# theartful/polychase

Hardware: AMD Instinct MI355X
Metric: optical-flow frames/sec (higher is better)
Workload: dtype u8/int32 fixed-point + f32 2x2 solve; 1 GPU; C2 1920x1080 300-frame synthetic clip, 3-level pyramidal LK (max_level=3); width=1920, height=1080, max_level=3, window=10, pairs_per_frame=8, frames_per_gpu=1877, arith=opencv_x86, parallelism=single GPU

## Files before the change

polychase_amd/csrc/hip/kernels_gftt.hip:

```cpp
#include <algorithm>
#include <cstring>
#include <type_traits>
#include <rocprim/device/device_radix_sort.hpp>

#include <cmath>

#include "kernels.hpp"

namespace pc {

constexpr int TW = 64, TH = 16;
constexpr int CW = TW + 2, CH = TH + 2;

constexpr int ME_R = 8;
constexpr int ME_TW = 64, ME_TH = 2 * ME_R;

template <int SOBEL, bool MASKED>
__global__ __launch_bounds__(256) void min_eig_fused_kernel(const uint8_t* __restrict__ img, int pitch, int w, int h,
                                                            float* __restrict__ eig, GfttGrid g,
                                                            uint32_t* __restrict__ cell_max, float f1, float f0, int hi_prio,
                                                            const uint8_t* __restrict__ mask) {
    helper_priority(hi_prio);
    const int lane = threadIdx.x & 63, wave = threadIdx.x >> 6;
    const int tx0 = (blockIdx.x * 2 + (wave & 1)) * ME_TW, ty0 = (blockIdx.y * 2 + (wave >> 1)) * ME_TH;
    if (tx0 >= w || ty0 >= h) return;
    const int x = tx0 + 2 * (lane & 31), y0 = ty0 + ME_R * (lane >> 5);
    const bool lane_on = x < w && y0 < h;
    const int cx_lo = tx0 / g.cell_w, cx_hi = min(tx0 + ME_TW - 1, w - 1) / g.cell_w;
    const int cy_lo = ty0 / g.cell_h, cy_hi = min(ty0 + ME_TH - 1, h - 1) / g.cell_h;
    const bool one_cell = cx_lo == cx_hi && cy_lo == cy_hi;
    const bool four_regs = !one_cell && g.cell_w >= ME_TW && g.cell_h >= ME_TH;
    const int bx = (cx_lo + 1) * g.cell_w, by = (cy_lo + 1) * g.cell_h;
    uint32_t kmax[4] = {0u, 0u, 0u, 0u};
    const bool edge_tile = tx0 == 0 || ty0 == 0 || tx0 + ME_TW + 1 > w || ty0 + ME_TH + 1 > h;

    auto walk = [&](auto edge_tag) {
        constexpr bool edge = decltype(edge_tag)::value;
        const int a = (x - 2) & ~3;
        const uint32_t o8 = (uint32_t)(x - 2 - a) * 8u;
        const uint8_t* col = img + a;
        const int cw = w - (x - 1);
        float rx[3][4], ry[3][4];
        double hprev[3][2], acc[3][2];
        auto emit = [&](int y, const double (&sv)[3][2]) {
            float e[2];
#pragma unroll
            for (int j = 0; j < 2; j++) {
                const float a2 = (float)sv[0][j] * 0.5f;
                const float b2 = (float)sv[1][j];
                const float c2 = (float)sv[2][j] * 0.5f;
                const float t = a2 - c2;
                e[j] = (a2 + c2) - sqrtf(t * t + b2 * b2);
            }
            float* out = eig + (size_t)y * w + x;
            const bool two = x + 1 < w;
            if (two && ((w & 1) == 0)) {
                *reinterpret_cast<float2*>(out) = make_float2(e[0], e[1]);
            } else {
                out[0] = e[0];
                if (two) out[1] = e[1];
            }
            uint32_t k0 = float_to_ordered(e[0]), k1 = two ? float_to_ordered(e[1]) : 0u;
            if (MASKED) {
                const uint8_t* m = mask + (size_t)y * w + x;
                if ((w & 1) == 0) {
                    const uint32_t mm = *reinterpret_cast<const uint16_t*>(m);
                    if ((mm & 0xffu) == 0) k0 = 0u;
                    if ((mm >> 8) == 0) k1 = 0u;
                } else {
                    if (m[0] == 0) k0 = 0u;
                    if (two && m[1] == 0) k1 = 0u;
                }
            }
            if (one_cell) {
                kmax[0] = max(kmax[0], max(k0, k1));
            } else if (four_regs) {
                const int qy = y >= by ? 2 : 0;
#pragma unroll
                for (int q = 0; q < 4; q++) {
                    const uint32_t v0 = (qy + (x >= bx ? 1 : 0)) == q ? k0 : 0u;
                    const uint32_t v1 = (qy + (x + 1 >= bx ? 1 : 0)) == q ? k1 : 0u;
                    kmax[q] = max(kmax[q], max(v0, v1));
                }
            } else {
                atomicMax(&cell_max[(y / g.cell_h) * g.cols + x / g.cell_w], k0);
                if (two) atomicMax(&cell_max[(y / g.cell_h) * g.cols + (x + 1) / g.cell_w], k1);
            }
        };
#pragma unroll
        for (int k = 0; k < ME_R + 4; k++) {
            const int gy = min(y0 - 2 + k, h);
            const uint32_t d0 = *reinterpret_cast<const uint32_t*>(col + (ptrdiff_t)gy * pitch);
            const uint32_t d1 = *reinterpret_cast<const uint32_t*>(col + (ptrdiff_t)gy * pitch + 4);
            const uint32_t lo = __builtin_amdgcn_alignbit(d1, d0, o8), hi = d1 >> o8;
            float gv[6];
            gv[0] = (float)(lo & 0xffu);
            gv[1] = (float)((lo >> 8) & 0xffu);
// ... 229 lines not shown
                                                           const uint8_t* __restrict__ mask) {
    helper_priority(hi_prio);
    const int x = blockIdx.x * 64 + (threadIdx.x & 63), y = blockIdx.y * 4 + (threadIdx.x >> 6);
    if (x >= w || y >= h) return;
    const size_t n = (size_t)w * h;
    const int a0 = block / 2;
    double sxx = 0, sxy = 0, syy = 0;
    if (rows) {
        for (int j = 0; j < block; j++) {
            const size_t at = (size_t)reflect101(y + j - a0, h) * w + x;
            sxx += rows[at];
            sxy += rows[n + at];
            syy += rows[2 * n + at];
        }
    } else {
        for (int j = 0; j < block; j++) {
            const size_t row = (size_t)reflect101(y + j - a0, h) * w;
            double rxx = 0, rxy = 0, ryy = 0;
            for (int i = 0; i < block; i++) {
                const size_t at = row + reflect101(x + i - a0, w);
                rxx += (double)cov[at];
                rxy += (double)cov[n + at];
                ryy += (double)cov[2 * n + at];
            }
            sxx += rxx;
            sxy += rxy;
            syy += ryy;
        }
    }
    float e;
    if (harris) {
        const float a = (float)sxx, b = (float)sxy, c = (float)syy;
        const float ac = a * c, bb = b * b;
        const float det = ac - bb, tr = a + c;
        if (harris == 2 && x < (w / 4) * 4) {
            const float kt = (float)harris_k * tr;
            e = det - kt * tr;
        } else {
            e = (float)((double)det - harris_k * (double)tr * (double)tr);
        }
    } else {
        const float a = (float)sxx * 0.5f, b = (float)sxy, c = (float)syy * 0.5f;
        const float t = a - c;
        e = (a + c) - sqrtf(t * t + b * b);
    }
    eig[(size_t)y * w + x] = e;
    uint32_t key = float_to_ordered(e);
    if (MASKED && mask[(size_t)y * w + x] == 0) key = 0u;
    const int cell = (y / g.cell_h) * g.cols + x / g.cell_w;
    const int cell0 = __builtin_amdgcn_readfirstlane(cell);
    if (__all(cell == cell0)) {
#pragma unroll
        for (int d = 32; d >= 1; d >>= 1) key = max(key, (uint32_t)__shfl_xor((int)key, d));
        if ((threadIdx.x & 63) == (unsigned)(__ffsll((long long)__ballot(1)) - 1)) atomicMax(&cell_max[cell0], key);
    } else {
        atomicMax(&cell_max[cell], key);
    }
}

bool launch_corner_response(const Level& l0, float* eig, float* cov, double* box_rows, const GfttGrid& g, uint32_t* cell_max, int block_size, int gradient_size,
                            bool harris, double harris_k, int sobel_fma, hipStream_t s, const uint8_t* mask) {
    SobelTaps T;
    int taps = 0;
    if (!make_sobel_taps(gradient_size, block_size, &T, &taps)) return false;
    dim3 grid((l0.w + 63) / 64, (l0.h + 3) / 4);
    if (taps == 3)
        hipLaunchKernelGGL(cov_kernel<3>, grid, dim3(256), 0, s, l0.img, l0.pitch, l0.w, l0.h, cov, T, sobel_fma, helper_prio_arg());
    else if (taps == 5)
        hipLaunchKernelGGL(cov_kernel<5>, grid, dim3(256), 0, s, l0.img, l0.pitch, l0.w, l0.h, cov, T, sobel_fma, helper_prio_arg());
    else
        hipLaunchKernelGGL(cov_kernel<7>, grid, dim3(256), 0, s, l0.img, l0.pitch, l0.w, l0.h, cov, T, sobel_fma, helper_prio_arg());
    if (box_rows) hipLaunchKernelGGL(box_rows_kernel, grid, dim3(256), 0, s, cov, l0.w, l0.h, block_size, box_rows, helper_prio_arg());
    const int harris_mode = harris ? ((sobel_fma & 1) ? 2 : 1) : 0;
    if (mask)
        hipLaunchKernelGGL(box_response_kernel<true>, grid, dim3(256), 0, s, cov, (const double*)box_rows, l0.w, l0.h, block_size, harris_mode, harris_k, eig, g, cell_max,
                           helper_prio_arg(), mask);
    else
        hipLaunchKernelGGL(box_response_kernel<false>, grid, dim3(256), 0, s, cov, (const double*)box_rows, l0.w, l0.h, block_size, harris_mode, harris_k, eig, g, cell_max,
                           helper_prio_arg(), (const uint8_t*)nullptr);
    return true;
}

constexpr int NMS_SUB = 4;

struct SortRange {
    uint32_t hi, shift;
};
__host__ __device__ __forceinline__ SortRange make_sort_range(uint32_t lo, uint32_t hi) {
    SortRange r;
    r.hi = hi;
    r.shift = 0;
    const uint32_t span = hi > lo ? hi - lo : 0u;
    while ((span >> r.shift) >= (uint32_t)kSortBuckets) r.shift++;
    return r;
}
__device__ __forceinline__ uint32_t bucket_of(uint32_t ord, const SortRange& r) {
    const uint32_t d = r.hi > ord ? r.hi - ord : 0u;
    const uint32_t b = d >> r.shift;
    return b < (uint32_t)kSortBuckets ? b : (uint32_t)kSortBuckets - 1u;
}

template <bool MASKED>
__global__ __launch_bounds__(256) void nms_kernel(const float* __restrict__ eig, int w, int h, GfttGrid g,
                                                  const uint32_t* __restrict__ cell_max, double quality_level,
                                                  unsigned long long* __restrict__ keys, uint32_t cap,
                                                  uint32_t* __restrict__ counter, uint8_t* __restrict__ cstate,
                                                  uint32_t* __restrict__ sort_params, uint32_t* __restrict__ hist,
                                                  uint32_t* __restrict__ ticket, uint32_t* __restrict__ bucket_offsets,
                                                  uint32_t* __restrict__ bin_hist, int n_tiles,
                                                  unsigned long long* __restrict__ slots, uint32_t* __restrict__ zero, int zero_words,
                                                  int hi_prio, const uint8_t* __restrict__ mask) {
    helper_priority(hi_prio);
    __shared__ float s_thr[kMaxGridCells];
    __shared__ uint32_t s_hi, s_lo;
    __shared__ float s_v[CH][CW + 2];
    __shared__ uint32_t s_wave[4];
    __shared__ uint32_t s_base;
    const int tid = threadIdx.x;
    const int x0 = blockIdx.x * TW;
    const int ncells = g.rows * g.cols;
    if (tid == 0) {
        s_hi = 0u;
        s_lo = 0xffffffffu;
    }
    __syncthreads();
    for (int i = tid; i < ncells; i += 256) {
        const float mx = (MASKED && cell_max[i] == 0u) ? 0.f : ordered_to_float(cell_max[i]);
        s_thr[i] = (float)((double)mx * quality_level);
        atomicMax(&s_hi, cell_max[i]);
        atomicMin(&s_lo, float_to_ordered(s_thr[i] > 0.f ? s_thr[i] : 0.f));
    }
    __syncthreads();
    const SortRange range = make_sort_range(s_lo, s_hi);
    if (blockIdx.x == 0 && blockIdx.y == 0) {
        if (tid == 0) {
            sort_params[0] = range.hi;
            sort_params[1] = range.shift;
        }
        if (bin_hist)
            for (int i = tid; i < n_tiles; i += 256) bin_hist[i] = 0u;
    }
    for (int i = (blockIdx.y * gridDim.x + blockIdx.x) * 256 + tid; i < zero_words; i += gridDim.x * gridDim.y * 256) zero[i] = 0u;
    const int r = tid >> 4, q = tid & 15;
    const int x = x0 + 4 * q;
    uint32_t flags = 0;
    float vals[NMS_SUB][4];
#pragma unroll
    for (int sub = 0; sub < NMS_SUB; sub++) {
        const int y0 = (blockIdx.y * NMS_SUB + sub) * TH;
        const int y = y0 + r;
        __syncthreads();
        const bool big_cells = g.cell_w >= CW && g.cell_h >= CH;
        const int ccx0 = max(x0 - 1, 0) / g.cell_w, ccy0 = max(y0 - 1, 0) / g.cell_h;
        const int bx = (ccx0 + 1) * g.cell_w, by = (ccy0 + 1) * g.cell_h;
        auto thr_at = [&](int ax, int ay) -> float {
            const int cx = big_cells ? ccx0 + (ax >= bx) : ax / g.cell_w;
            const int cy = big_cells ? ccy0 + (ay >= by) : ay / g.cell_h;
            return s_thr[cy * g.cols + cx];
        };
        if (y0 < h) {
            float v[4] = {0.f, 0.f, 0.f, 0.f};
            if (y < h && x < w) {
                const float* row = eig + (size_t)y * w;
                if (x + 3 < w && (w & 3) == 0) {
                    const float4 e = *reinterpret_cast<const float4*>(row + x);
                    v[0] = e.x; v[1] = e.y; v[2] = e.z; v[3] = e.w;
                } else {
                    for (int i = 0; i < 4 && x + i < w; i++) v[i] = row[x + i];
                }
#pragma unroll
                for (int i = 0; i < 4; i++) v[i] = (x + i < w && v[i] > thr_at(x + i, y)) ? v[i] : 0.f;
            }
#pragma unroll
            for (int i = 0; i < 4; i++) s_v[r + 1][4 * q + 1 + i] = v[i];
            if (tid < 2 * CW + 2 * TH) {
                int cx, cy;
                if (tid < 2 * CW) {
                    cy = tid < CW ? 0 : CH - 1;
                    cx = tid < CW ? tid : tid - CW;
                } else {
                    const int k = tid - 2 * CW;
                    cy = 1 + (k >> 1);
                    cx = (k & 1) ? CW - 1 : 0;
                }
                const int ax = x0 - 1 + cx, ay = y0 - 1 + cy;
                float e = 0.f;
                if (ax >= 0 && ax < w && ay >= 0 && ay < h) {
                    e = eig[(size_t)ay * w + ax];
                    e = (e > thr_at(ax, ay)) ? e : 0.f;
                }
                s_v[cy][cx] = e;
            }
        }
        __syncthreads();
#pragma unroll
        for (int i = 0; i < 4; i++) vals[sub][i] = 0.f;
        if (y < h && x < w) {
            float cm[6];
#pragma unroll
            for (int i = 0; i < 6; i++) {
                const float a = s_v[r][4 * q + i], b = s_v[r + 1][4 * q + i], c = s_v[r + 2][4 * q + i];
                const float m = a > b ? a : b;
                cm[i] = m > c ? m : c;
            }
            uint32_t f4 = 0;
            uint32_t on = 0xfu;
            if (MASKED) {
                const uint8_t* mk = mask + (size_t)y * w + x;
                uint32_t m4 = 0;
                if (x + 3 < w && ((w & 3) == 0)) {
                    m4 = *reinterpret_cast<const uint32_t*>(mk);
                } else {
                    for (int i = 0; i < 4 && x + i < w; i++) m4 |= (uint32_t)mk[i] << (8 * i);
                }
                on = ((m4 & 0xffu) ? 1u : 0u) | ((m4 & 0xff00u) ? 2u : 0u) | ((m4 & 0xff0000u) ? 4u : 0u) | ((m4 & 0xff000000u) ? 8u : 0u);
            }
#pragma unroll
            for (int i = 0; i < 4; i++) {
                const float val = s_v[r + 1][4 * q + 1 + i];
                float m = cm[i] > cm[i + 1] ? cm[i] : cm[i + 1];
                m = m > cm[i + 2] ? m : cm[i + 2];
                const int xi = x + i;
                if (val != 0.f && val == m && xi >= 1 && xi < w - 1 && y >= 1 && y < h - 1 && (!MASKED || ((on >> i) & 1u))) {
                    f4 |= 1u << i;
                    vals[sub][i] = val;
                }
            }
            flags |= f4 << (4 * sub);
            uint8_t* cs = cstate + (size_t)y * w + x;
            if (x + 3 < w && ((w & 3) == 0)) {
                *reinterpret_cast<uint32_t*>(cs) = (f4 & 1u) | ((f4 & 2u) << 7) | ((f4 & 4u) << 14) | ((f4 & 8u) << 21);
            } else {
                for (int i = 0; i < 4 && x + i < w; i++) cs[i] = (uint8_t)((f4 >> i) & 1u);
            }
        }
    }
    const int lane = tid & 63, wave = tid >> 6;
    const uint32_t cnt = (uint32_t)__popc(flags);
    uint32_t incl = cnt;
#pragma unroll
    for (int d = 1; d < 64; d <<= 1) {
        const uint32_t t = __shfl_up(incl, d);
        if (lane >= d) incl += t;
    }
    if (lane == 63) s_wave[wave] = incl;
    __syncthreads();
    if (tid == 0) {
        const uint32_t total = s_wave[0] + s_wave[1] + s_wave[2] + s_wave[3];
        s_base = total ? atomicAdd(counter, total) : 0u;
    }
    __syncthreads();
    if (cnt != 0) {
        uint32_t pos = s_base + incl - cnt;
        for (int wv = 0; wv < wave; wv++) pos += s_wave[wv];
#pragma unroll
        for (int sub = 0; sub < NMS_SUB; sub++) {
            const int y = (blockIdx.y * NMS_SUB + sub) * TH + r;
#pragma unroll
            for (int i = 0; i < 4; i++) {
                if (flags & (1u << (4 * sub + i))) {
                    const uint32_t ord = float_to_ordered(vals[sub][i]);
                    if (pos < cap) {
                        const unsigned long long key = ((unsigned long long)ord << 32) | (unsigned long long)(uint32_t)(y * w + x + i);
                        const uint32_t b = bucket_of(ord, range);
                        if (slots) {
                            const uint32_t at = atomicAdd(&hist[b], 1u);
                            slots[(size_t)b * kBucketSlots + min(at, (uint32_t)kBucketSlots - 1u)] = key;
                        } else {
                            keys[pos] = key;
                            atomicAdd(&hist[b], 1u);
                        }
                    }
                    pos++;
                }
            }
        }
    }
    if (ticket && last_workgroup(ticket, gridDim.x * gridDim.y)) {
        __shared__ uint32_t s_scan[256];
        const uint32_t total = scan_exclusive_256_fixed<kSortBuckets / 256>(hist, bucket_offsets, s_scan);
        if (tid == 0) bucket_offsets[kSortBuckets] = total;
    }
}

void launch_nms(const float* eig, int w, int h, const GfttGrid& g, const uint32_t* cell_max, double quality_level,
                unsigned long long* keys, uint32_t cap, uint32_t* counter, uint8_t* cstate, uint32_t* sort_params, uint32_t* hist,
                uint32_t* ticket, uint32_t* bucket_offsets, uint32_t* bin_hist, hipStream_t s,
                unsigned long long* slots, uint32_t* zero, int zero_words, const uint8_t* mask) {
    dim3 grid((w + TW - 1) / TW, (h + NMS_SUB * TH - 1) / (NMS_SUB * TH));
    if (mask)
        hipLaunchKernelGGL(nms_kernel<true>, grid, dim3(256), 0, s, eig, w, h, g, cell_max, quality_level, keys, cap, counter, cstate,
                           sort_params, hist, ticket, bucket_offsets, bin_hist, bin_hist ? bin_num_tiles(w, h) : 0, slots, zero,
                           zero ? zero_words : 0, helper_prio_arg(), mask);
    else
        hipLaunchKernelGGL(nms_kernel<false>, grid, dim3(256), 0, s, eig, w, h, g, cell_max, quality_level, keys, cap, counter, cstate,
                           sort_params, hist, ticket, bucket_offsets, bin_hist, bin_hist ? bin_num_tiles(w, h) : 0, slots, zero,
                           zero ? zero_words : 0, helper_prio_arg(), (const uint8_t*)nullptr);
}

constexpr int kBucketLds = 512;

__global__ __launch_bounds__(256) void bucket_scatter_kernel(const unsigned long long* __restrict__ keys, uint32_t cap,
                                                             const uint32_t* __restrict__ counter, const uint32_t* __restrict__ sort_params,
                                                             const uint32_t* __restrict__ offsets, uint32_t* __restrict__ cursor,
                                                             unsigned long long* __restrict__ out, int hi_prio) {
    helper_priority(hi_prio);
    const uint32_t n = min(*counter, cap);
    SortRange range;
    range.hi = sort_params[0];
    range.shift = sort_params[1];
    for (uint32_t i = blockIdx.x * blockDim.x + threadIdx.x; i < n; i += gridDim.x * blockDim.x) {
        const unsigned long long key = keys[i];
        const uint32_t b = bucket_of((uint32_t)(key >> 32), range);
        out[offsets[b] + atomicAdd(&cursor[b], 1u)] = key;
    }
}

constexpr int kBucketsPerWave = 4;

constexpr int kSortWaves = 4;
static_assert(kBucketSlots == kBucketLds, "a bucket beyond its slots is a bucket beyond the fast path");
template <bool SLOTS>
__global__ __launch_bounds__(64 * kSortWaves) void bucket_sort_kernel(const unsigned long long* __restrict__ in, const uint32_t* __restrict__ offsets,
                                                         unsigned long long* __restrict__ out, uint32_t* __restrict__ overflow, int hi_prio) {
    helper_priority(hi_prio);
    __shared__ unsigned long long s_all[kSortWaves][kBucketLds];
    const int lane = threadIdx.x & 63, wave = threadIdx.x >> 6;
    unsigned long long* const s_keys = s_all[wave];
    const int b0 = (blockIdx.x * kSortWaves + wave) * kBucketsPerWave;
    if (b0 >= kSortBuckets) return;
    uint32_t o[kBucketsPerWave + 1];
#pragma unroll
    for (int k = 0; k <= kBucketsPerWave; k++) o[k] = offsets[min(b0 + k, kSortBuckets)];
    const uint32_t lo = o[0], n4 = o[kBucketsPerWave] - lo;
    if (n4 == 0) return;
    if (n4 <= (uint32_t)kBucketLds) {
        unsigned long long ld[kBucketLds / 64];
#pragma unroll
        for (int q = 0; q < kBucketLds / 64; q++) {
            const uint32_t i = lane + 64 * q;
            size_t at = lo + i;
            if (SLOTS) {
                int k = 0;
#pragma unroll
                for (int kk = 1; kk < kBucketsPerWave; kk++)
                    if (lo + i >= o[kk]) k = kk;
                at = (size_t)(b0 + k) * kBucketSlots + (lo + i - o[k]);
            }
            ld[q] = i < n4 ? in[at] : 0ull;
        }
#pragma unroll
        for (int q = 0; q < kBucketLds / 64; q++) {
            const uint32_t i = lane + 64 * q;
            if (i < n4) s_keys[i] = ld[q];
        }
        __builtin_amdgcn_fence(__ATOMIC_ACQ_REL, "wavefront");
        uint32_t longest = 0;
#pragma unroll
// ... 2 lines not shown
            const unsigned long long mine = s_keys[i];
            uint32_t a = lo, b = o[1];
#pragma unroll
            for (int k = 1; k < kBucketsPerWave; k++)
                if (lo + i >= o[k]) {
                    a = o[k];
                    b = o[k + 1];
                }
            const uint32_t first = a - lo, len = b - a;
            uint32_t rank = 0;
#pragma unroll 8
            for (uint32_t j = 0; j < longest; j++) {
                const unsigned long long other = s_keys[first + min(j, len - 1u)];
                rank += (j < len && other > mine) ? 1u : 0u;
            }
            out[a + rank] = mine;
        }
        return;
    }
    for (int b = b0; b < b0 + kBucketsPerWave && b < kSortBuckets; b++) {
        const uint32_t base = offsets[b], n = offsets[b + 1] - base;
        const unsigned long long* const src = SLOTS ? in + (size_t)b * kBucketSlots : in + base;
        if (n == 0) continue;
        if (n > (uint32_t)kBucketLds) {
            if (lane == 0) atomicOr(overflow, 1u);
            for (uint32_t i = lane; i < n; i += 64) out[base + i] = src[SLOTS ? min(i, (uint32_t)kBucketSlots - 1u) : i];
            continue;
        }
        __builtin_amdgcn_fence(__ATOMIC_ACQ_REL, "wavefront");
        for (uint32_t i = lane; i < n; i += 64) s_keys[i] = src[i];
        __builtin_amdgcn_fence(__ATOMIC_ACQ_REL, "wavefront");
        for (uint32_t i = lane; i < n; i += 64) {
            const unsigned long long mine = s_keys[i];
            uint32_t rank = 0;
#pragma unroll 8
            for (uint32_t j = 0; j < n; j++) rank += s_keys[j] > mine ? 1u : 0u;
            out[base + rank] = mine;
        }
    }
}

void launch_bucket_sort(const unsigned long long* keys, uint32_t cap, uint32_t n_launch, const uint32_t* counter, const uint32_t* sort_params,
                        const uint32_t* offsets, uint32_t* cursor, unsigned long long* scratch, unsigned long long* out,
                        uint32_t* overflow, hipStream_t s) {
    const unsigned blocks = std::max(1u, std::min<unsigned>(1024u, (n_launch + 255u) / 256u));
    hipLaunchKernelGGL(bucket_scatter_kernel, dim3(blocks), dim3(256), 0, s, keys, cap, counter, sort_params, offsets, cursor, scratch, helper_prio_arg());
    hipLaunchKernelGGL(bucket_sort_kernel<false>, dim3((kSortBuckets / kBucketsPerWave + kSortWaves - 1) / kSortWaves), dim3(64 * kSortWaves), 0, s, scratch,
                       offsets, out, overflow, helper_prio_arg());
}
void launch_bucket_sort_slots(const unsigned long long* slots, const uint32_t* offsets, unsigned long long* out, uint32_t* overflow,
                              hipStream_t s) {
    hipLaunchKernelGGL(bucket_sort_kernel<true>, dim3((kSortBuckets / kBucketsPerWave + kSortWaves - 1) / kSortWaves), dim3(64 * kSortWaves), 0, s, slots,
                       offsets, out, overflow, helper_prio_arg());
}

struct AcceptedScan {
    uint32_t* ticket;
    uint32_t* n_out;
    uint32_t* overflow;
    uint32_t max_corners;
};
__device__ __forceinline__ void finish_accepted_scan(uint32_t* per_block, const AcceptedScan& fin, uint32_t n_max, const uint32_t* n_dev) {
    if (!last_workgroup(fin.ticket, gridDim.x)) return;
    __shared__ uint32_t s_scan[256];
    if (threadIdx.x == 0 && n_dev && fin.overflow && *n_dev > n_max) atomicOr(fin.overflow, 4u);
    const uint32_t total = scan_exclusive_256(per_block, per_block, (int)gridDim.x, s_scan);
    if (threadIdx.x == 0) *fin.n_out = (fin.max_corners > 0 && total > fin.max_corners) ? fin.max_corners : total;
}

constexpr uint8_t CS_CAND = 1, CS_ACCEPTED = 2, CS_REJECTED = 3;
constexpr int SUP_NB = 12;
constexpr int SUP_BLOCK = 256;

__device__ __forceinline__ uint8_t cs_load(const uint8_t* p) { return __hip_atomic_load(p, __ATOMIC_RELAXED, __HIP_MEMORY_SCOPE_AGENT); }
__device__ __forceinline__ void cs_store(uint8_t* p, uint8_t v) { __hip_atomic_store(p, v, __ATOMIC_RELAXED, __HIP_MEMORY_SCOPE_AGENT); }

__device__ __forceinline__ bool suppress_decide(const unsigned long long* __restrict__ keys, uint32_t n, int w, int h,
                                                const float* __restrict__ eig, uint8_t* cstate, const int2* __restrict__ offsets,
                                                int n_offsets, const int* __restrict__ row_hw, int R, uint32_t* __restrict__ stuck,
                                                uint32_t* idx_out) {
    const uint32_t i = blockIdx.x * SUP_BLOCK + threadIdx.x;
    const bool live = i < n;
    uint32_t my_val = 0, my_idx = 0;
    uint32_t nb[SUP_NB];
    int n_nb = 0;
    bool overflow = false;
    int x = 0, y = 0;
    if (live) {
        const unsigned long long key = keys[i];
        my_val = (uint32_t)(key >> 32);
        my_idx = (uint32_t)key;
        y = (int)(my_idx / (uint32_t)w);
        x = (int)(my_idx - (uint32_t)y * (uint32_t)w);
        for (int dy = -R; dy <= R; dy++) {
            const int ny = y + dy, hw = row_hw[dy + R];
            if (ny < 0 || ny >= h || hw < 0) continue;
            const uint32_t lin0 = (uint32_t)(ny * w + max(x - hw, 0)), lin1 = (uint32_t)(ny * w + min(x + hw, w - 1));
            for (uint32_t a = lin0 & ~3u; a <= lin1; a += 4u) {
                uint32_t v = *reinterpret_cast<const uint32_t*>(cstate + a);
                if (a < lin0) v &= 0xffffffffu << (8u * (lin0 - a));
                if (a + 3u > lin1) v &= 0xffffffffu >> (8u * (a + 3u - lin1));
                while (v) {
                    const uint32_t b = (uint32_t)(__ffs((int)v) - 1) >> 3;
                    v &= ~(0xffu << (8u * b));
                    const uint32_t nidx = a + b;
                    if (nidx == my_idx) continue;
                    const uint32_t nval = float_to_ordered(eig[nidx]);
                    if (!(nval > my_val || (nval == my_val && nidx > my_idx))) continue;
                    if (n_nb < SUP_NB) {
#pragma unroll
                        for (int k = 0; k < SUP_NB; k++)
                            if (k == n_nb) nb[k] = nidx;
                        n_nb++;
                    } else {
                        overflow = true;
                    }
                }
            }
        }
    }
    bool done = !live;
    bool accepted = false;
    for (uint32_t spin = 0;; spin++) {
        if (!done) {
            bool blocked = false, rejected = false;
            if (overflow) {
                for (int o = 0; o < n_offsets; o++) {
                    const int nx = x + offsets[o].x, ny = y + offsets[o].y;
                    if (nx < 0 || nx >= w || ny < 0 || ny >= h) continue;
                    const uint32_t nidx = (uint32_t)(ny * w + nx);
                    const uint8_t st = cs_load(&cstate[nidx]);
                    if (st == 0) continue;
                    const uint32_t nval = float_to_ordered(eig[nidx]);
                    if (!(nval > my_val || (nval == my_val && nidx > my_idx))) continue;
                    rejected |= (st == CS_ACCEPTED);
                    blocked |= (st == CS_CAND);
                }
            } else {
#pragma unroll
                for (int k = 0; k < SUP_NB; k++) {
                    if (k < n_nb) {
                        const uint8_t st = cs_load(&cstate[nb[k]]);
                        rejected |= (st == CS_ACCEPTED);
                        blocked |= (st == CS_CAND);
                    }
                }
            }
            if (rejected || !blocked) {
                cs_store(&cstate[my_idx], rejected ? CS_REJECTED : CS_ACCEPTED);
                accepted = !rejected;
                done = true;
            }
        }
        if (__all(done)) break;
        if (spin > (1u << 22)) {
            if (!done) atomicAdd(stuck, 1u);
            break;
        }
        __builtin_amdgcn_s_sleep(1);
    }
    *idx_out = my_idx;
    return accepted;
}

__global__ __launch_bounds__(SUP_BLOCK) void suppress_sorted_kernel(const unsigned long long* __restrict__ keys, uint32_t n_max,
                                                                    const uint32_t* __restrict__ n_dev, int w, int h,
                                                                    const float* __restrict__ eig, uint8_t* cstate,
                                                                    const int2* __restrict__ offsets, int n_offsets,
                                                                    const int* __restrict__ row_hw, int R,
                                                                    uint32_t* __restrict__ accepted_per_block,
                                                                    uint32_t* __restrict__ stuck, AcceptedScan fin, int hi_prio) {
    helper_priority(hi_prio);
    const uint32_t n = n_dev ? min(*n_dev, n_max) : n_max;
    uint32_t idx;
    const bool accepted = suppress_decide(keys, n, w, h, eig, cstate, offsets, n_offsets, row_hw, R, stuck, &idx);
    const int c = __syncthreads_count(accepted);
    if (threadIdx.x == 0) publish(&accepted_per_block[blockIdx.x], (uint32_t)c);
    finish_accepted_scan(accepted_per_block, fin, n_max, n_dev);
}

constexpr uint32_t kLbAggregate = 1u << 30, kLbPrefix = 1u << 31, kLbCount = kLbAggregate - 1u;
__device__ __forceinline__ uint32_t lookback_exclusive(uint32_t* lookback, uint32_t b, uint32_t c, uint32_t* __restrict__ stuck) {
    const int lane = (int)(threadIdx.x & 63);
    if (b == 0) {
        if (lane == 0) publish(&lookback[0], kLbPrefix | c);
        return 0u;
    }
    if (lane == 0) publish(&lookback[b], kLbAggregate | c);
    uint32_t excl = 0;
    int top = (int)b - 1;
    for (uint32_t spin = 0;; spin++) {
        const int j = top - lane;
        const uint32_t v = j >= 0 ? __hip_atomic_load(&lookback[j], __ATOMIC_RELAXED, __HIP_MEMORY_SCOPE_AGENT) : kLbPrefix;
        const unsigned long long pre = __ballot((v & kLbPrefix) != 0u);
        const int stop = pre ? __ffsll((long long)pre) - 1 : 63;
// ... 252 lines not shown
```

polychase_amd/csrc/hip/kernels_pyramid.hip:

```cpp
#include "kernels.hpp"

namespace pc {

static thread_local int tl_helper_prio = 0;
int helper_prio_arg() { return tl_helper_prio; }
void set_helper_prio(int hi) { tl_helper_prio = hi ? 1 : 0; }

namespace {

constexpr int TW = 64, TH = 16;
constexpr int CW = TW + 2, CH = TH + 2;
constexpr int C_X0 = 3;
constexpr int C_PITCH = 72;
constexpr int P_H = 2 * TH + 7;
constexpr int P_PITCH = 144;
constexpr int H_Q = (CW + 3) / 4;
constexpr int H_PITCH = 4 * H_Q;

__device__ __forceinline__ uint32_t gray_of(uint32_t r, uint32_t g, uint32_t b) {
    return (r * 9798u + g * 19235u + b * 3735u + (1u << 14)) >> 15;
}
__device__ __forceinline__ uint32_t float_channel_to_u8(float v) {
    const float s = v * 255.0f;
    const int i = (s >= -2147483648.0f && s < 2147483648.0f) ? (int)s : (int)0x80000000;
    return (uint32_t)i & 0xffu;
}

template <int SRC>
__device__ __forceinline__ uint32_t gray_src(const LevelSource& in, uint32_t r, uint32_t g, uint32_t b) {
    if constexpr (SRC == SRC_RGB8_W || SRC == SRC_RGBF32_W || SRC == SRC_RGBF32_T) return (r * in.wr + g * in.wg + b * in.wb + (1u << 14)) >> 15;
    else return gray_of(r, g, b);
}
template <int SRC>
__device__ __forceinline__ uint32_t float_channel(const LevelSource& in, const float* s) {
    if constexpr (SRC == SRC_RGBF32_T) return in.table[transfer_index(*reinterpret_cast<const uint32_t*>(s))];
    else return float_channel_to_u8(*s);
}

template <int SRC>
__device__ __forceinline__ uint32_t source_gray(const LevelSource& in, int x, int y) {
    const uint8_t* row = in.src + (size_t)y * in.src_pitch;
    if (SRC == SRC_RGB8 || SRC == SRC_RGB8_W) {
        const uint8_t* s = row + 3 * (size_t)x;
        return gray_src<SRC>(in, s[0], s[1], s[2]);
    } else if (SRC == SRC_GRAY8) {
        return row[x];
    } else {
        const float* s = reinterpret_cast<const float*>(row) + (size_t)x * in.channels;
        return gray_src<SRC>(in, float_channel<SRC>(in, s), float_channel<SRC>(in, s + 1), float_channel<SRC>(in, s + 2));
    }
}

constexpr int kNone = -(1 << 30);
__device__ __forceinline__ void mirrors(int v, int len, int win, int m[3]) {
    m[0] = v;
    m[1] = (v >= 1 && v <= win) ? -v : kNone;
    m[2] = (v <= len - 2 && v >= len - 1 - win) ? 2 * (len - 1) - v : kNone;
}

}

template <int SRC>
__global__ __launch_bounds__(256) void level_kernel(const LevelSource in, const Level out, const int win, int hi_prio) {
    helper_priority(hi_prio);
    __shared__ __attribute__((aligned(16))) uint8_t s_c[CH][C_PITCH];
    __shared__ __attribute__((aligned(16))) uint8_t s_p[SRC == SRC_PYR ? P_H : 1][P_PITCH];
    __shared__ __attribute__((aligned(16))) uint16_t s_h[SRC == SRC_PYR ? P_H : 1][H_PITCH];

    const int tid = threadIdx.x;
    const int x0 = blockIdx.x * TW, y0 = blockIdx.y * TH;
    const int w = out.w, h = out.h;
    if (in.clear) {
        const int stride = (int)(gridDim.x * gridDim.y) * 256;
        for (int i = (int)(blockIdx.y * gridDim.x + blockIdx.x) * 256 + tid; i < in.clear_words; i += stride) in.clear[i] = 0u;
    }

    if constexpr (SRC == SRC_PYR) {
        const Level& P = in.parent;
        const int px0 = 2 * x0 - 4, py0 = 2 * y0 - 4;
        const int ymin = -win, ymax = P.h + win - 1, xmax = P.pitch - kPadX - 4;
        for (int i = tid; i < P_H * (P_PITCH / 4); i += 256) {
            const int r = i / (P_PITCH / 4), d = i - r * (P_PITCH / 4);
            const int yy = min(max(py0 + r, ymin), ymax), xx = min(px0 + 4 * d, xmax);
            *reinterpret_cast<uint32_t*>(&s_p[r][4 * d]) = *reinterpret_cast<const uint32_t*>(P.img + (ptrdiff_t)yy * P.pitch + xx);
        }
        __syncthreads();
        for (int i = tid; i < P_H * H_Q; i += 256) {
            const int r = i / H_Q, q = i - r * H_Q;
            const uint32_t* p = reinterpret_cast<const uint32_t*>(&s_p[r][8 * q]);
            const uint32_t a = p[0], b = p[1], c = p[2];
            int v[11];
            v[0] = a & 0xff; v[1] = (a >> 8) & 0xff; v[2] = (a >> 16) & 0xff; v[3] = a >> 24;
            v[4] = b & 0xff; v[5] = (b >> 8) & 0xff; v[6] = (b >> 16) & 0xff; v[7] = b >> 24;
            v[8] = c & 0xff; v[9] = (c >> 8) & 0xff; v[10] = (c >> 16) & 0xff;
            uint32_t o[4];
#pragma unroll
            for (int k = 0; k < 4; k++) o[k] = (uint32_t)(v[2 * k + 2] * 6 + (v[2 * k + 1] + v[2 * k + 3]) * 4 + v[2 * k] + v[2 * k + 4]);
            *reinterpret_cast<uint2*>(&s_h[r][4 * q]) = make_uint2(o[0] | (o[1] << 16), o[2] | (o[3] << 16));
        }
        __syncthreads();
        for (int i = tid; i < CH * (H_PITCH / 2); i += 256) {
            const int cy = i / (H_PITCH / 2), cp = i - cy * (H_PITCH / 2);
            const int c = 2 * cp;
            if (c >= CW) continue;
            uint32_t t[5];
#pragma unroll
            for (int k = 0; k < 5; k++) t[k] = *reinterpret_cast<const uint32_t*>(&s_h[2 * cy + k][c]);
            const uint32_t lo = ((t[0] & 0xffff) + (t[4] & 0xffff) + ((t[1] & 0xffff) + (t[3] & 0xffff)) * 4 + (t[2] & 0xffff) * 6 + 128) >> 8;
            const uint32_t hi = ((t[0] >> 16) + (t[4] >> 16) + ((t[1] >> 16) + (t[3] >> 16)) * 4 + (t[2] >> 16) * 6 + 128) >> 8;
            s_c[cy][C_X0 + c] = (uint8_t)lo;
            if (c + 1 < CW) s_c[cy][C_X0 + c + 1] = (uint8_t)hi;
        }
    } else {
        const int r = tid >> 4, g = tid & 15;
        const int x = x0 + 4 * g, y = y0 + r;
        if (y < h && x < w) {
            uint32_t px[4] = {0, 0, 0, 0};
            if (in.aligned && x + 3 < w) {
                const uint8_t* row = in.src + (size_t)y * in.src_pitch;
                if (SRC == SRC_RGB8 || SRC == SRC_RGB8_W) {
                    const uint32_t* s = reinterpret_cast<const uint32_t*>(row) + 3 * (x >> 2);
                    const uint32_t d0 = s[0], d1 = s[1], d2 = s[2];
                    px[0] = gray_src<SRC>(in, d0 & 0xff, (d0 >> 8) & 0xff, (d0 >> 16) & 0xff);
                    px[1] = gray_src<SRC>(in, d0 >> 24, d1 & 0xff, (d1 >> 8) & 0xff);
                    px[2] = gray_src<SRC>(in, (d1 >> 16) & 0xff, d1 >> 24, d2 & 0xff);
                    px[3] = gray_src<SRC>(in, (d2 >> 8) & 0xff, (d2 >> 16) & 0xff, d2 >> 24);
                } else if (SRC == SRC_GRAY8) {
                    const uint32_t d = *reinterpret_cast<const uint32_t*>(row + x);
                    px[0] = d & 0xff; px[1] = (d >> 8) & 0xff; px[2] = (d >> 16) & 0xff; px[3] = d >> 24;
                } else {
#pragma unroll
                    for (int k = 0; k < 4; k++) px[k] = source_gray<SRC>(in, x + k, y);
                }
            } else {
#pragma unroll
                for (int k = 0; k < 4; k++)
                    if (x + k < w) px[k] = source_gray<SRC>(in, x + k, y);
            }
            *reinterpret_cast<uint32_t*>(&s_c[r + 1][C_X0 + 1 + 4 * g]) = px[0] | (px[1] << 8) | (px[2] << 16) | (px[3] << 24);
        }
        if (tid < 2 * CW + 2 * TH) {
            int cx, cy;
            if (tid < 2 * CW) {
                cy = tid < CW ? 0 : CH - 1;
                cx = tid < CW ? tid : tid - CW;
            } else {
                const int k = tid - 2 * CW;
                cy = 1 + (k >> 1);
                cx = (k & 1) ? CW - 1 : 0;
            }
            const int ax = x0 - 1 + cx, ay = y0 - 1 + cy;
            if (ax >= 0 && ax < w && ay >= 0 && ay < h) s_c[cy][C_X0 + cx] = (uint8_t)source_gray<SRC>(in, ax, ay);
        }
    }
    __syncthreads();
    const bool edge_tile = x0 == 0 || y0 == 0 || x0 + TW >= w || y0 + TH >= h;
    if (edge_tile) {
        for (int i = tid; i < CW * CH; i += 256) {
            const int cy = i / CW, cx = i - cy * CW;
            const int ax = x0 - 1 + cx, ay = y0 - 1 + cy;
            if ((ax < 0 || ax >= w || ay < 0 || ay >= h) && ax >= -1 && ax <= w && ay >= -1 && ay <= h) {
                const int sx = reflect101(ax, w) - (x0 - 1), sy = reflect101(ay, h) - (y0 - 1);
                if (sx >= 0 && sx < CW && sy >= 0 && sy < CH) s_c[cy][C_X0 + cx] = s_c[sy][C_X0 + sx];
            }
        }
        __syncthreads();
    }

    const int r = tid >> 4, g = tid & 15;
    const int x = x0 + 4 * g, y = y0 + r;
    if (y >= h || x >= w) return;
    uint32_t rows[3][3];
#pragma unroll
    for (int k = 0; k < 3; k++) {
        const uint32_t* p = reinterpret_cast<const uint32_t*>(&s_c[r + k][4 * g]);
        rows[k][0] = p[0];
        rows[k][1] = p[1];
        rows[k][2] = p[2];
    }
    const uint32_t centre = rows[1][1];
    int t0[6], t1[6];
#pragma unroll
    for (int i = 0; i < 6; i++) {
        const int sh = 8 * ((3 + i) & 3), wd = (3 + i) >> 2;
        const int a = (rows[0][wd] >> sh) & 0xff, c = (rows[1][wd] >> sh) & 0xff, b = (rows[2][wd] >> sh) & 0xff;
        t0[i] = (a + b) * 3 + c * 10;
        t1[i] = b - a;
    }
    int32_t d[4];
#pragma unroll
    for (int i = 0; i < 4; i++) {
        const int dx = t0[i + 2] - t0[i];
        const int dy = (t1[i + 2] + t1[i]) * 3 + t1[i + 1] * 10;
        d[i] = (int32_t)((uint32_t)(dx & 0xffff) | ((uint32_t)(dy & 0xffff) << 16));
    }
    const uint32_t w16lo = __builtin_amdgcn_perm(0u, centre, 0x0c010c00u) << 7;
    const uint32_t w16hi = __builtin_amdgcn_perm(0u, centre, 0x0c030c02u) << 7;
    uint8_t* img = out.img + (ptrdiff_t)y * out.pitch + x;
    uint16_t* img16 = out.img16 + (ptrdiff_t)y * out.pitch + x;
    int32_t* der = out.der + (ptrdiff_t)y * out.pitch + x;
    if (x + 3 < w) {
        *reinterpret_cast<uint32_t*>(img) = centre;
        *reinterpret_cast<uint2*>(img16) = make_uint2(w16lo, w16hi);
        *reinterpret_cast<int4*>(der) = make_int4(d[0], d[1], d[2], d[3]);
    } else {
        for (int i = 0; i < 4 && x + i < w; i++) {
            const uint32_t v = (centre >> (8 * i)) & 0xff;
            img[i] = (uint8_t)v;
            img16[i] = (uint16_t)(v << 7);
            der[i] = d[i];
        }
    }
    if (x <= win || x + 3 >= w - 1 - win || y <= win || y >= h - 1 - win) {
        int my[3];
        mirrors(y, h, win, my);
        for (int i = 0; i < 4 && x + i < w; i++) {
            const uint32_t v = (centre >> (8 * i)) & 0xff;
            int mx[3];
            mirrors(x + i, w, win, mx);
#pragma unroll
            for (int a = 0; a < 3; a++)
#pragma unroll
                for (int b = 0; b < 3; b++) {
                    if ((a | b) == 0 || my[a] == kNone || mx[b] == kNone) continue;
                    const ptrdiff_t o = (ptrdiff_t)my[a] * out.pitch + mx[b];
                    out.img[o] = (uint8_t)v;
                    out.img16[o] = (uint16_t)(v << 7);
                }
        }
    }
}

void launch_level(const LevelSource& in, const Level& out, int win, hipStream_t s) {
    dim3 grid((out.w + TW - 1) / TW, (out.h + TH - 1) / TH);
    switch (in.kind) {
        case SRC_PYR: hipLaunchKernelGGL(level_kernel<SRC_PYR>, grid, dim3(256), 0, s, in, out, win, helper_prio_arg()); break;
        case SRC_RGB8: hipLaunchKernelGGL(level_kernel<SRC_RGB8>, grid, dim3(256), 0, s, in, out, win, helper_prio_arg()); break;
        case SRC_GRAY8: hipLaunchKernelGGL(level_kernel<SRC_GRAY8>, grid, dim3(256), 0, s, in, out, win, helper_prio_arg()); break;
        case SRC_RGB8_W: hipLaunchKernelGGL(level_kernel<SRC_RGB8_W>, grid, dim3(256), 0, s, in, out, win, helper_prio_arg()); break;
        case SRC_RGBF32_W: hipLaunchKernelGGL(level_kernel<SRC_RGBF32_W>, grid, dim3(256), 0, s, in, out, win, helper_prio_arg()); break;
        case SRC_RGBF32_T: hipLaunchKernelGGL(level_kernel<SRC_RGBF32_T>, grid, dim3(256), 0, s, in, out, win, helper_prio_arg()); break;
        default: hipLaunchKernelGGL(level_kernel<SRC_RGBF32>, grid, dim3(256), 0, s, in, out, win, helper_prio_arg()); break;
    }
}

}
```

Measured before the change: 3425 frames/s.

## Restructure NMS tiling, vectorize Scharr derivatives, and drop parent-row LDS staging

Several independent changes land together. Min-eig tile height grows (ME_R 8→10). NMS now processes two 16-row tiles per shared-memory fill with a block-wide early-out when all values are zero, uses integer compares when no threshold is negative, and reloads the eig value at emit time instead of holding it in registers. The suppression neighbour scan tests 16 bytes per step using a bitmask. The pyramid level kernel reads parent rows directly from global memory instead of staging them in LDS, and computes the Scharr derivatives with packed 16-bit vector math. Together these aim to cut syncs, registers and ALU work, at the cost of redundant global loads and more complex code.

```diff
diff --git a/polychase_amd/csrc/hip/kernels_gftt.hip b/polychase_amd/csrc/hip/kernels_gftt.hip
--- a/polychase_amd/csrc/hip/kernels_gftt.hip
+++ b/polychase_amd/csrc/hip/kernels_gftt.hip
@@ -12,7 +12,7 @@
 constexpr int TW = 64, TH = 16;
 constexpr int CW = TW + 2, CH = TH + 2;
 
-constexpr int ME_R = 8;
+constexpr int ME_R = 10;
 constexpr int ME_TW = 64, ME_TH = 2 * ME_R;
 
 template <int SOBEL, bool MASKED>
@@ -408,6 +408,8 @@
 }
 
 constexpr int NMS_SUB = 4;
+constexpr int NMS_PART = 2;
+constexpr int kNmsPartBoundaries = (NMS_PART * TH + 1) / CH + 1;
 
 struct SortRange {
     uint32_t hi, shift;
@@ -438,8 +440,8 @@
                                                   int hi_prio, const uint8_t* __restrict__ mask) {
     helper_priority(hi_prio);
     __shared__ float s_thr[kMaxGridCells];
-    __shared__ uint32_t s_hi, s_lo;
-    __shared__ float s_v[CH][CW + 2];
+    __shared__ uint32_t s_hi, s_lo, s_neg;
+    __shared__ float s_v[NMS_PART * TH + 2][CW + 2];
     __shared__ uint32_t s_wave[4];
     __shared__ uint32_t s_base;
     const int tid = threadIdx.x;
@@ -448,6 +450,7 @@
     if (tid == 0) {
         s_hi = 0u;
         s_lo = 0xffffffffu;
+        s_neg = 0u;
     }
     __syncthreads();
     for (int i = tid; i < ncells; i += 256) {
@@ -455,6 +458,7 @@
         s_thr[i] = (float)((double)mx * quality_level);
         atomicMax(&s_hi, cell_max[i]);
         atomicMin(&s_lo, float_to_ordered(s_thr[i] > 0.f ? s_thr[i] : 0.f));
+        if (__float_as_uint(s_thr[i]) >> 31) atomicOr(&s_neg, 1u);
     }
     __syncthreads();
     const SortRange range = make_sort_range(s_lo, s_hi);
@@ -469,98 +473,147 @@
     for (int i = (blockIdx.y * gridDim.x + blockIdx.x) * 256 + tid; i < zero_words; i += gridDim.x * gridDim.y * 256) zero[i] = 0u;
     const int r = tid >> 4, q = tid & 15;
     const int x = x0 + 4 * q;
+    const bool in_x = x < w;
+    const bool quad = x + 3 < w && (w & 3) == 0;
+    const bool big_cells = g.cell_w >= CW && g.cell_h >= CH;
+    const int ccx0 = max(x0 - 1, 0) / g.cell_w, bx = (ccx0 + 1) * g.cell_w;
     uint32_t flags = 0;
-    float vals[NMS_SUB][4];
-#pragma unroll
-    for (int sub = 0; sub < NMS_SUB; sub++) {
-        const int y0 = (blockIdx.y * NMS_SUB + sub) * TH;
-        const int y = y0 + r;
-        __syncthreads();
-        const bool big_cells = g.cell_w >= CW && g.cell_h >= CH;
-        const int ccx0 = max(x0 - 1, 0) / g.cell_w, ccy0 = max(y0 - 1, 0) / g.cell_h;
-        const int bx = (ccx0 + 1) * g.cell_w, by = (ccy0 + 1) * g.cell_h;
+    auto stencil = [&](auto ordered_tag, auto sub_tag, const bool any_value) {
+        constexpr bool ORDERED = decltype(ordered_tag)::value;
+        constexpr int sub = decltype(sub_tag)::value, lr = (sub % NMS_PART) * TH;
+        using T = std::conditional_t<ORDERED, uint32_t, float>;
+        const int y = (blockIdx.y * NMS_SUB + sub) * TH + r;
+        if (!(y < h && in_x)) return;
+        uint32_t f4 = 0;
+        if (any_value) {
+            const T(*sv)[CW + 2] = reinterpret_cast<const T(*)[CW + 2]>(s_v);
+            T cm[6];
+#pragma unroll
+            for (int i = 0; i < 6; i++) {
+                const T a = sv[lr + r][4 * q + i], b = sv[lr + r + 1][4 * q + i], c = sv[lr + r + 2][4 * q + i];
+                if constexpr (ORDERED) {
+                    cm[i] = max(max(a, b), c);
+                } else {
+                    const T m = a > b ? a : b;
+                    cm[i] = m > c ? m : c;
+                }
+            }
+            uint32_t on = 0xfu;
+            if (MASKED) {
+                const uint8_t* mk = mask + (size_t)y * w + x;
+                uint32_t m4 = 0;
+                if (quad) {
+                    m4 = *reinterpret_cast<const uint32_t*>(mk);
+                } else {
+                    for (int i = 0; i < 4 && x + i < w; i++) m4 |= (uint32_t)mk[i] << (8 * i);
+                }
+                on = ((m4 & 0xffu) ? 1u : 0u) | ((m4 & 0xff00u) ? 2u : 0u) | ((m4 & 0xff0000u) ? 4u : 0u) | ((m4 & 0xff000000u) ? 8u : 0u);
+            }
+            if (!(y >= 1 && y < h - 1)) on = 0u;
+#pragma unroll
+            for (int i = 0; i < 4; i++) {
+                const T val = sv[lr + r + 1][4 * q + 1 + i];
+                T m;
+                if constexpr (ORDERED) {
+                    m = max(max(cm[i], cm[i + 1]), cm[i + 2]);
+                } else {
+                    m = cm[i] > cm[i + 1] ? cm[i] : cm[i + 1];
+                    m = m > cm[i + 2] ? m : cm[i + 2];
+                }
+                const int xi = x + i;
+                if (val != (T)0 && val == m && xi >= 1 && xi < w - 1 && ((on >> i) & 1u)) f4 |= 1u << i;
+            }
+            flags |= f4 << (4 * sub);
+        }
+        uint8_t* cs = cstate + (size_t)y * w + x;
+        if (quad) {
+            *reinterpret_cast<uint32_t*>(cs) = (f4 & 1u) | ((f4 & 2u) << 7) | ((f4 & 4u) << 14) | ((f4 & 8u) << 21);
+        } else {
+            for (int i = 0; i < 4 && x + i < w; i++) cs[i] = (uint8_t)((f4 >> i) & 1u);
+        }
+    };
+    auto part = [&](auto part_tag) {
+        constexpr int P = decltype(part_tag)::value;
+        const int yp = (blockIdx.y * NMS_SUB + P * NMS_PART) * TH;
+        if (yp >= h) return;
+        const int cyb = max(yp - 1, 0) / g.cell_h;
         auto thr_at = [&](int ax, int ay) -> float {
-            const int cx = big_cells ? ccx0 + (ax >= bx) : ax / g.cell_w;
-            const int cy = big_cells ? ccy0 + (ay >= by) : ay / g.cell_h;
+            int cx, cy;
+            if (big_cells) {
+                cx = ccx0 + (ax >= bx);
+                cy = cyb;
+#pragma unroll
+                for (int k = 1; k <= kNmsPartBoundaries; k++) cy += ay >= (cyb + k) * g.cell_h;
+            } else {
+                cx = ax / g.cell_w;
+                cy = ay / g.cell_h;
+            }
             return s_thr[cy * g.cols + cx];
         };
-        if (y0 < h) {
+        if (P > 0) __syncthreads();
+        uint32_t nz = 0u;
+#pragma unroll
+        for (int t = 0; t < NMS_PART; t++) {
+            const int y0 = yp + t * TH;
+            const int y = y0 + r;
             float v[4] = {0.f, 0.f, 0.f, 0.f};
-            if (y < h && x < w) {
+            if (y < h && in_x) {
                 const float* row = eig + (size_t)y * w;
-                if (x + 3 < w && (w & 3) == 0) {
+                if (quad) {
                     const float4 e = *reinterpret_cast<const float4*>(row + x);
                     v[0] = e.x; v[1] = e.y; v[2] = e.z; v[3] = e.w;
                 } else {
                     for (int i = 0; i < 4 && x + i < w; i++) v[i] = row[x + i];
                 }
-#pragma unroll
-                for (int i = 0; i < 4; i++) v[i] = (x + i < w && v[i] > thr_at(x + i, y)) ? v[i] : 0.f;
-            }
-#pragma unroll
-            for (int i = 0; i < 4; i++) s_v[r + 1][4 * q + 1 + i] = v[i];
-            if (tid < 2 * CW + 2 * TH) {
-                int cx, cy;
-                if (tid < 2 * CW) {
-                    cy = tid < CW ? 0 : CH - 1;
-                    cx = tid < CW ? tid : tid - CW;
+                if (big_cells) {
+                    const int ccy0 = max(y0 - 1, 0) / g.cell_h;
+                    const float* trow = &s_thr[(ccy0 + (y >= (ccy0 + 1) * g.cell_h)) * g.cols + ccx0];
+                    const float t_lo = trow[0], t_hi = trow[min(x + 3, w - 1) >= bx ? 1 : 0];
+#pragma unroll
+                    for (int i = 0; i < 4; i++) v[i] = v[i] > (x + i >= bx ? t_hi : t_lo) ? v[i] : 0.f;
                 } else {
-                    const int k = tid - 2 * CW;
-                    cy = 1 + (k >> 1);
-                    cx = (k & 1) ? CW - 1 : 0;
-                }
-                const int ax = x0 - 1 + cx, ay = y0 - 1 + cy;
-                float e = 0.f;
-                if (ax >= 0 && ax < w && ay >= 0 && ay < h) {
-                    e = eig[(size_t)ay * w + ax];
-                    e = (e > thr_at(ax, ay)) ? e : 0.f;
-                }
-                s_v[cy][cx] = e;
-            }
-        }
-        __syncthreads();
-#pragma unroll
-        for (int i = 0; i < 4; i++) vals[sub][i] = 0.f;
-        if (y < h && x < w) {
-            float cm[6];
-#pragma unroll
-            for (int i = 0; i < 6; i++) {
-                const float a = s_v[r][4 * q + i], b = s_v[r + 1][4 * q + i], c = s_v[r + 2][4 * q + i];
-                const float m = a > b ? a : b;
-                cm[i] = m > c ? m : c;
-            }
-            uint32_t f4 = 0;
-            uint32_t on = 0xfu;
-            if (MASKED) {
-                const uint8_t* mk = mask + (size_t)y * w + x;
-                uint32_t m4 = 0;
-                if (x + 3 < w && ((w & 3) == 0)) {
-                    m4 = *reinterpret_cast<const uint32_t*>(mk);
-                } else {
-                    for (int i = 0; i < 4 && x + i < w; i++) m4 |= (uint32_t)mk[i] << (8 * i);
-                }
-                on = ((m4 & 0xffu) ? 1u : 0u) | ((m4 & 0xff00u) ? 2u : 0u) | ((m4 & 0xff0000u) ? 4u : 0u) | ((m4 & 0xff000000u) ? 8u : 0u);
+#pragma unroll
+                    for (int i = 0; i < 4; i++) v[i] = (x + i < w && v[i] > thr_at(x + i, y)) ? v[i] : 0.f;
+                }
             }
 #pragma unroll
             for (int i = 0; i < 4; i++) {
-                const float val = s_v[r + 1][4 * q + 1 + i];
-                float m = cm[i] > cm[i + 1] ? cm[i] : cm[i + 1];
-                m = m > cm[i + 2] ? m : cm[i + 2];
-                const int xi = x + i;
-                if (val != 0.f && val == m && xi >= 1 && xi < w - 1 && y >= 1 && y < h - 1 && (!MASKED || ((on >> i) & 1u))) {
-                    f4 |= 1u << i;
-                    vals[sub][i] = val;
-                }
-            }
-            flags |= f4 << (4 * sub);
-            uint8_t* cs = cstate + (size_t)y * w + x;
-            if (x + 3 < w && ((w & 3) == 0)) {
-                *reinterpret_cast<uint32_t*>(cs) = (f4 & 1u) | ((f4 & 2u) << 7) | ((f4 & 4u) << 14) | ((f4 & 8u) << 21);
+                s_v[t * TH + r + 1][4 * q + 1 + i] = v[i];
+                nz |= __float_as_uint(v[i]) << 1;
+            }
+        }
+        static_assert(2 * CW + 2 * NMS_PART * TH <= 256, "one ring position per lane");
+        if (tid < 2 * CW + 2 * NMS_PART * TH) {
+            int cx, cy;
+            if (tid < 2 * CW) {
+                cy = tid < CW ? 0 : NMS_PART * TH + 1;
+                cx = tid < CW ? tid : tid - CW;
             } else {
-                for (int i = 0; i < 4 && x + i < w; i++) cs[i] = (uint8_t)((f4 >> i) & 1u);
-            }
-        }
-    }
+                const int j = tid - 2 * CW;
+                cy = 1 + (j >> 1);
+                cx = (j & 1) ? CW - 1 : 0;
+            }
+            const int ax = x0 - 1 + cx, ay = yp - 1 + cy;
+            float e = 0.f;
+            if (ax >= 0 && ax < w && ay >= 0 && ay < h) {
+                e = eig[(size_t)ay * w + ax];
+                e = (e > thr_at(ax, ay)) ? e : 0.f;
+            }
+            s_v[cy][cx] = e;
+            nz |= __float_as_uint(e) << 1;
+        }
+        const bool any_value = __syncthreads_or(nz != 0u) != 0;
+        auto tiles = [&](auto ordered_tag) {
+            stencil(ordered_tag, std::integral_constant<int, P * NMS_PART>{}, any_value);
+            stencil(ordered_tag, std::integral_constant<int, P * NMS_PART + 1>{}, any_value);
+        };
+        static_assert(NMS_PART == 2, "two stencils per part");
+        if (s_neg == 0u) tiles(std::true_type{});
+        else tiles(std::false_type{});
+    };
+    part(std::integral_constant<int, 0>{});
+    part(std::integral_constant<int, 1>{});
+    static_assert(NMS_SUB == 2 * NMS_PART, "two parts per block");
     const int lane = tid & 63, wave = tid >> 6;
     const uint32_t cnt = (uint32_t)__popc(flags);
     uint32_t incl = cnt;
@@ -579,27 +632,22 @@
     if (cnt != 0) {
         uint32_t pos = s_base + incl - cnt;
         for (int wv = 0; wv < wave; wv++) pos += s_wave[wv];
-#pragma unroll
-        for (int sub = 0; sub < NMS_SUB; sub++) {
-            const int y = (blockIdx.y * NMS_SUB + sub) * TH + r;
-#pragma unroll
-            for (int i = 0; i < 4; i++) {
-                if (flags & (1u << (4 * sub + i))) {
-                    const uint32_t ord = float_to_ordered(vals[sub][i]);
-                    if (pos < cap) {
-                        const unsigned long long key = ((unsigned long long)ord << 32) | (unsigned long long)(uint32_t)(y * w + x + i);
-                        const uint32_t b = bucket_of(ord, range);
-                        if (slots) {
-                            const uint32_t at = atomicAdd(&hist[b], 1u);
-                            slots[(size_t)b * kBucketSlots + min(at, (uint32_t)kBucketSlots - 1u)] = key;
-                        } else {
-                            keys[pos] = key;
-                            atomicAdd(&hist[b], 1u);
-                        }
-                    }
-                    pos++;
-                }
-            }
+        for (uint32_t todo = flags; todo != 0u; todo &= todo - 1u) {
+            const int bit = __ffs((int)todo) - 1;
+            const uint32_t idx = (uint32_t)(((blockIdx.y * NMS_SUB + (bit >> 2)) * TH + r) * w + x + (bit & 3));
+            const uint32_t ord = float_to_ordered(eig[idx]);
+            if (pos < cap) {
+                const unsigned long long key = ((unsigned long long)ord << 32) | (unsigned long long)idx;
+                const uint32_t b = bucket_of(ord, range);
+                if (slots) {
+                    const uint32_t at = atomicAdd(&hist[b], 1u);
+                    slots[(size_t)b * kBucketSlots + min(at, (uint32_t)kBucketSlots - 1u)] = key;
+                } else {
+                    keys[pos] = key;
+                    atomicAdd(&hist[b], 1u);
+                }
+            }
+            pos++;
         }
     }
     if (ticket && last_workgroup(ticket, gridDim.x * gridDim.y)) {
@@ -768,7 +816,7 @@
     const uint32_t i = blockIdx.x * SUP_BLOCK + threadIdx.x;
     const bool live = i < n;
     uint32_t my_val = 0, my_idx = 0;
-    uint32_t nb[SUP_NB];
+    uint32_t nb[SUP_NB] = {};
     int n_nb = 0;
     bool overflow = false;
     int x = 0, y = 0;
@@ -782,21 +830,24 @@
             const int ny = y + dy, hw = row_hw[dy + R];
             if (ny < 0 || ny >= h || hw < 0) continue;
             const uint32_t lin0 = (uint32_t)(ny * w + max(x - hw, 0)), lin1 = (uint32_t)(ny * w + min(x + hw, w - 1));
-            for (uint32_t a = lin0 & ~3u; a <= lin1; a += 4u) {
-                uint32_t v = *reinterpret_cast<const uint32_t*>(cstate + a);
-                if (a < lin0) v &= 0xffffffffu << (8u * (lin0 - a));
-                if (a + 3u > lin1) v &= 0xffffffffu >> (8u * (a + 3u - lin1));
-                while (v) {
-                    const uint32_t b = (uint32_t)(__ffs((int)v) - 1) >> 3;
-                    v &= ~(0xffu << (8u * b));
-                    const uint32_t nidx = a + b;
+            for (uint32_t a0 = lin0 & ~3u; a0 <= lin1; a0 += 16u) {
+                uint32_t vv[4];
+#pragma unroll
+                for (int j = 0; j < 4; j++) vv[j] = a0 + 4u * j <= lin1 ? *reinterpret_cast<const uint32_t*>(cstate + a0 + 4u * j) : 0u;
+                uint32_t m = 0;
+#pragma unroll
+                for (int j = 0; j < 4; j++) m |= ((((vv[j] | (vv[j] >> 1)) & 0x01010101u) * 0x01020408u) >> 24 & 0xfu) << (4 * j);
+                if (a0 < lin0) m &= 0xffffu << (lin0 - a0);
+                if (a0 + 15u > lin1) m &= 0xffffu >> (a0 + 15u - lin1);
+                for (; m != 0u; m &= m - 1u) {
+                    const uint32_t nidx = a0 + (uint32_t)(__ffs((int)m) - 1);
                     if (nidx == my_idx) continue;
                     const uint32_t nval = float_to_ordered(eig[nidx]);
                     if (!(nval > my_val || (nval == my_val && nidx > my_idx))) continue;
                     if (n_nb < SUP_NB) {
 #pragma unroll
-                        for (int k = 0; k < SUP_NB; k++)
-                            if (k == n_nb) nb[k] = nidx;
+                        for (int k = SUP_NB - 1; k > 0; k--) nb[k] = nb[k - 1];
+                        nb[0] = nidx;
                         n_nb++;
                     } else {
                         overflow = true;
diff --git a/polychase_amd/csrc/hip/kernels_pyramid.hip b/polychase_amd/csrc/hip/kernels_pyramid.hip
--- a/polychase_amd/csrc/hip/kernels_pyramid.hip
+++ b/polychase_amd/csrc/hip/kernels_pyramid.hip
@@ -13,7 +13,6 @@
 constexpr int C_X0 = 3;
 constexpr int C_PITCH = 72;
 constexpr int P_H = 2 * TH + 7;
-constexpr int P_PITCH = 144;
 constexpr int H_Q = (CW + 3) / 4;
 constexpr int H_PITCH = 4 * H_Q;
 
@@ -64,7 +63,6 @@
 __global__ __launch_bounds__(256) void level_kernel(const LevelSource in, const Level out, const int win, int hi_prio) {
     helper_priority(hi_prio);
     __shared__ __attribute__((aligned(16))) uint8_t s_c[CH][C_PITCH];
-    __shared__ __attribute__((aligned(16))) uint8_t s_p[SRC == SRC_PYR ? P_H : 1][P_PITCH];
     __shared__ __attribute__((aligned(16))) uint16_t s_h[SRC == SRC_PYR ? P_H : 1][H_PITCH];
 
     const int tid = threadIdx.x;
@@ -79,16 +77,13 @@
         const Level& P = in.parent;
         const int px0 = 2 * x0 - 4, py0 = 2 * y0 - 4;
         const int ymin = -win, ymax = P.h + win - 1, xmax = P.pitch - kPadX - 4;
-        for (int i = tid; i < P_H * (P_PITCH / 4); i += 256) {
-            const int r = i / (P_PITCH / 4), d = i - r * (P_PITCH / 4);
-            const int yy = min(max(py0 + r, ymin), ymax), xx = min(px0 + 4 * d, xmax);
-            *reinterpret_cast<uint32_t*>(&s_p[r][4 * d]) = *reinterpret_cast<const uint32_t*>(P.img + (ptrdiff_t)yy * P.pitch + xx);
-        }
-        __syncthreads();
         for (int i = tid; i < P_H * H_Q; i += 256) {
             const int r = i / H_Q, q = i - r * H_Q;
-            const uint32_t* p = reinterpret_cast<const uint32_t*>(&s_p[r][8 * q]);
-            const uint32_t a = p[0], b = p[1], c = p[2];
+            const int yy = min(max(py0 + r, ymin), ymax);
+            const uint8_t* prow = P.img + (ptrdiff_t)yy * P.pitch;
+            const uint32_t a = *reinterpret_cast<const uint32_t*>(prow + min(px0 + 8 * q, xmax));
+            const uint32_t b = *reinterpret_cast<const uint32_t*>(prow + min(px0 + 8 * q + 4, xmax));
+            const uint32_t c = *reinterpret_cast<const uint32_t*>(prow + min(px0 + 8 * q + 8, xmax));
             int v[11];
             v[0] = a & 0xff; v[1] = (a >> 8) & 0xff; v[2] = (a >> 16) & 0xff; v[3] = a >> 24;
             v[4] = b & 0xff; v[5] = (b >> 8) & 0xff; v[6] = (b >> 16) & 0xff; v[7] = b >> 24;
@@ -179,20 +174,30 @@
         rows[k][2] = p[2];
     }
     const uint32_t centre = rows[1][1];
-    int t0[6], t1[6];
-#pragma unroll
-    for (int i = 0; i < 6; i++) {
-        const int sh = 8 * ((3 + i) & 3), wd = (3 + i) >> 2;
-        const int a = (rows[0][wd] >> sh) & 0xff, c = (rows[1][wd] >> sh) & 0xff, b = (rows[2][wd] >> sh) & 0xff;
-        t0[i] = (a + b) * 3 + c * 10;
-        t1[i] = b - a;
+    typedef uint16_t u16x2 __attribute__((ext_vector_type(2)));
+    u16x2 pr[3][3];
+#pragma unroll
+    for (int k = 0; k < 3; k++) {
+        pr[k][0] = __builtin_bit_cast(u16x2, __builtin_amdgcn_perm(rows[k][1], rows[k][0], 0x0c040c03u));
+        pr[k][1] = __builtin_bit_cast(u16x2, __builtin_amdgcn_perm(0u, rows[k][1], 0x0c020c01u));
+        pr[k][2] = __builtin_bit_cast(u16x2, __builtin_amdgcn_perm(rows[k][2], rows[k][1], 0x0c040c03u));
+    }
+    const u16x2 k3 = {3, 3}, k10 = {10, 10};
+    u16x2 t0[3], t1[3];
+#pragma unroll
+    for (int j = 0; j < 3; j++) {
+        t0[j] = (pr[0][j] + pr[2][j]) * k3 + pr[1][j] * k10;
+        t1[j] = pr[2][j] - pr[0][j];
     }
     int32_t d[4];
 #pragma unroll
-    for (int i = 0; i < 4; i++) {
-        const int dx = t0[i + 2] - t0[i];
-        const int dy = (t1[i + 2] + t1[i]) * 3 + t1[i + 1] * 10;
-        d[i] = (int32_t)((uint32_t)(dx & 0xffff) | ((uint32_t)(dy & 0xffff) << 16));
+    for (int j = 0; j < 2; j++) {
+        const u16x2 dx = t0[j + 1] - t0[j];
+        const u16x2 mid = __builtin_bit_cast(u16x2, __builtin_amdgcn_alignbit(__builtin_bit_cast(uint32_t, t1[j + 1]), __builtin_bit_cast(uint32_t, t1[j]), 16u));
+        const u16x2 dy = (t1[j + 1] + t1[j]) * k3 + mid * k10;
+        const uint32_t dxu = __builtin_bit_cast(uint32_t, dx), dyu = __builtin_bit_cast(uint32_t, dy);
+        d[2 * j] = (int32_t)__builtin_amdgcn_perm(dyu, dxu, 0x05040100u);
+        d[2 * j + 1] = (int32_t)__builtin_amdgcn_perm(dyu, dxu, 0x07060302u);
     }
     const uint32_t w16lo = __builtin_amdgcn_perm(0u, centre, 0x0c010c00u) << 7;
     const uint32_t w16hi = __builtin_amdgcn_perm(0u, centre, 0x0c030c02u) << 7;
```

Result: faster. 3518 frames/s (median of 6 runs) (+2.7%).
